# xxcclong/GNN-Computing

Measured on NVIDIA B200. Metric: gcn_layer_algorithmic_GBps, higher is better.
Workload: dtype f32

## Files before the change

### gnn-computing_b200/csrc/capi.cu

```cuda
#include <cuda_runtime.h>

#include <cstdio>
#include <cstdlib>
#include <cstring>
#include <memory>
#include <string>
#include <utility>
#include <vector>

#include "agg_kernels.cuh"
#include "edge_kernels.cuh"
#include "gnnagg.h"
#include "internal.h"

namespace gnnagg {

static thread_local std::string g_error;

int set_error(int code, const char *msg)
{
    g_error = msg ? msg : "";
    return code;
}

#define CUDA_TRY(expr)                                                                       \
    do {                                                                                     \
        cudaError_t _e = (expr);                                                             \
        if (_e != cudaSuccess) {                                                             \
            char _buf[512];                                                                  \
            snprintf(_buf, sizeof _buf, "%s:%d %s: %s", __FILE__, __LINE__, #expr, cudaGetErrorString(_e)); \
            return set_error(GNNAGG_ERR_CUDA, _buf);                                         \
        }                                                                                    \
    } while (0)

#define LAUNCH_CHECK(a)                   \
    do {                                  \
        CUDA_TRY(cudaPeekAtLastError()); \
        ++(a)->launches;                  \
    } while (0)

template <class T>
struct DevBuf {
    T *p = nullptr;
    size_t cap = 0;

    DevBuf() = default;
    DevBuf(const DevBuf &) = delete;
    DevBuf(DevBuf &&o) noexcept : p(o.p), cap(o.cap) { o.p = nullptr, o.cap = 0; }
    DevBuf &operator=(DevBuf o) noexcept
    {
        std::swap(p, o.p), std::swap(cap, o.cap);
        return *this;
    }
    ~DevBuf()
    {
        if (p) cudaFree(p);
    }

    int ensure(size_t need)
    {
        if (need <= cap && p) return GNNAGG_OK;
        if (p) CUDA_TRY(cudaFree(p));
        p = nullptr;
        cap = 0;
        CUDA_TRY(cudaMalloc((void **)&p, (need ? need : 1) * sizeof(T)));
        cap = need;
        return GNNAGG_OK;
    }
    void adopt(T *q) { *this = DevBuf(), p = q; }
};

template <int N>
struct Events {
    cudaEvent_t e[N] = {};

    Events() = default;
    Events(const Events &) = delete;
    ~Events()
    {
        for (cudaEvent_t x : e)
            if (x) cudaEventDestroy(x);
    }
    cudaEvent_t operator[](int i) const { return e[i]; }
    bool created() const { return e[0] != nullptr; }
    int create(unsigned flags)
    {
        for (cudaEvent_t &x : e) CUDA_TRY(cudaEventCreateWithFlags(&x, flags));
        return GNNAGG_OK;
    }
};

struct SideStream {
    cudaStream_t stream = nullptr;
    Events<9> ev;

    SideStream() = default;
    SideStream(const SideStream &) = delete;
    ~SideStream()
    {
        if (stream) cudaStreamDestroy(stream);
    }
    int ensure()
    {
        if (stream) return GNNAGG_OK;
        CUDA_TRY(cudaStreamCreateWithFlags(&stream, cudaStreamNonBlocking));
        return ev.create(cudaEventDisableTiming);
    }
};

static inline int64_t cdiv(int64_t a, int64_t b) { return (a + b - 1) / b; }

static bool pdl_enabled()
{
    static const bool on = [] {
        const char *e = getenv("GNNAGG_PDL");
        return e ? atoi(e) != 0 : true;
    }();
    return on;
}

template <class... KArgs, class... Args>
static void launch_dep(void (*kernel)(KArgs...), unsigned grid, unsigned block, cudaStream_t st, Args &&...args)
{
    cudaLaunchConfig_t cfg{};
    cfg.gridDim = dim3(grid);
    cfg.blockDim = dim3(block);
    cfg.stream = st;
    cudaLaunchAttribute attr[1];
    attr[0].id = cudaLaunchAttributeProgrammaticStreamSerialization;
    attr[0].val.programmaticStreamSerializationAllowed = 1;
    cfg.attrs = attr;
    cfg.numAttrs = pdl_enabled() ? 1 : 0;
    cudaLaunchKernelEx(&cfg, kernel, KArgs(args)...);
}

}

using namespace gnnagg;

constexpr int kMaxSlices = 16;
constexpr double kLocalityMinL2Multiples = 8.0;
constexpr double kLocalitySliceL2Multiples = 2.5;
constexpr double kLocalityMinDegree = 20.0;
constexpr int kLocalityMaxAuto = 4;
constexpr int64_t kMergeMinEdges = 4000000;
constexpr double kMergeMinFraction = 0.10;

struct LongRows {
    int item_edges = 0, count = 0;
    DevBuf<int> list;
    DevBuf<int2> records;
};

struct View {
    gnnagg_aggregator *root = nullptr;
    const int *d_ptr = nullptr, *d_idx = nullptr;
    const float *d_val = nullptr;
    int n = 0, m = 0;
    const int *d_item_row = nullptr;
    int num_items = 0;
    int warp_edges = 0;
    bool records = false;
    const int *out_row = nullptr;
    DevBuf<float> carry, carry_den, den_row;
    std::vector<LongRows> long_rows;
    const int *h_ptr_user = nullptr;
    std::vector<int> h_ptr;
};

struct Slices {
    struct Slice {
        DevBuf<int> item_row, c_ptr, out_row;
        View v;
    };
    DevBuf<int> ptr, idx, perm;
    DevBuf<float> val;
    uint64_t val_gen = 0;
    int off[kMaxSlices] = {0}, cnt[kMaxSlices] = {0};
    int width = 0;
    std::vector<Slice> slice;
};

struct Transpose {
    DevBuf<int> ptr, idx, perm, item_row;
    DevBuf<float> val;
    uint64_t val_gen = 0;
    View v;
};

struct Merged {
    DevBuf<int> ptr, idx, start, item_row;
    DevBuf<float> val;
    uint64_t val_gen = 0;
    View v;
};

struct Schedule {
    int kind = GNNAGG_SCHED_NOP;
    int num_target = 0, edges = 0, items = 0;
    DevBuf<int> ptr, target, perm, item_row, own_idx;
    DevBuf<float> own_val;
    const int *idx = nullptr;
    const float *val = nullptr;
};

struct gnnagg_aggregator : View {
    int64_t launches = 0;
    uint64_t val_gen = 0;
    DevBuf<int> item_row;
    DevBuf<float> newval, ax;
    DevBuf<float> st_in, st_out, st_w, st_att;
    Schedule sched;
    std::unique_ptr<Transpose> tr;
    DevBuf<float2> bwd_c, bwd_wt, bwd_part, bwd_carry;
    DevBuf<float> bwd_t;
    SideStream copy, in;
    int host_slices = 0;
    std::unique_ptr<Slices> host;
    int loc_slices = 0;
    std::unique_ptr<Slices> loc;
    int merge_mode = 0;
    int merge_auto = -1;
    std::unique_ptr<Merged> mg;
    bool prof = false;
    Events<5> ev;
};

#define PROF_RECORD(a, i, st)                                   \
    do {                                                        \
        if ((a)->prof) CUDA_TRY(cudaEventRecord((a)->ev[i], st)); \
    } while (0)

namespace gnnagg {

static EdgeParams edge_params(const View &v)
{
    EdgeParams g;
    g.ptr = v.d_ptr;
    g.idx = v.d_idx;
    g.item_row = v.d_item_row;
    g.num_rows = v.n;
    g.num_edges = v.m;
    g.num_items = v.num_items;
    return g;
}

int build_item_rows_device(const int *d_ptr, int rows, int edges, int **out, int *items, cudaStream_t st)
{
    *items = (int)cdiv(edges, kFineItem);
    *out = nullptr;
    CUDA_TRY(cudaMalloc((void **)out, (size_t)(*items ? *items : 1) * sizeof(int)));
    if (*items > 0) {
        item_row_kernel<<<(unsigned)cdiv(*items, 256), 256, 0, st>>>(d_ptr, rows, edges, *out, *items);
        CUDA_TRY(cudaPeekAtLastError());
    }
    return GNNAGG_OK;
}

static int item_table(DevBuf<int> &buf, const int *d_ptr, int rows, int edges, int *items, cudaStream_t st)
{
    int *out = nullptr;
    const int rc = build_item_rows_device(d_ptr, rows, edges, &out, items, st);
    buf.adopt(out);
    return rc;
}

__global__ void gather_val_kernel(const float *__restrict__ val, const int *__restrict__ perm, float *__restrict__ out,
                                  int count)
{
    const int i = blockIdx.x * blockDim.x + threadIdx.x;
    if (i < count) out[i] = __ldg(val + __ldg(perm + i));
}

__global__ void scatter_val_kernel(const float *__restrict__ in, const int *__restrict__ perm, float *__restrict__ out, int count)
{
    const int i = blockIdx.x * blockDim.x + threadIdx.x;
    if (i < count) out[__ldg(perm + i)] = __ldg(in + i);
}

__global__ void merge_val_kernel(const float *__restrict__ val, const int *__restrict__ start, float *__restrict__ out,
                                 int runs)
{
    const int k = blockIdx.x * blockDim.x + threadIdx.x;
    if (k >= runs) return;
    const int end = __ldg(start + k + 1);
    double s = 0.0;
    for (int e = __ldg(start + k); e < end; ++e) s += (double)__ldg(val + e);
    out[k] = (float)s;
}

static int check_feat(int F)
{
    if (F < 4 || F > 1024 || (F & 3)) return set_error(GNNAGG_ERR_ARG, "feat must be a multiple of 4 in [4,1024]");
    return GNNAGG_OK;
}

static inline int lanes_for(int F) { return F <= 32 ? 8 : (F <= 64 ? 16 : 32); }

constexpr int64_t kSmallGraphEdges = 4000000;

static inline int warp_edges_for(const View &v, int64_t num_edges)
{
    if (v.warp_edges) return v.warp_edges;
    return num_edges < kSmallGraphEdges ? 128 : kWarpEdges;
}
static inline int item_edges_for(const View &v, int F, int64_t num_edges)
{
    return warp_edges_for(v, num_edges) / (32 / lanes_for(F));
}

using AggKernel = void (*)(const AggParams);

template <int MODE, bool SCHED, bool XBF16 = false>
static AggKernel agg_kernel_for(int WE, int F)
{
    if (WE == 128)
        return F <= 32 ? agg_kernel<8, 1, MODE, SCHED, 128, XBF16>
             : F <= 64 ? agg_kernel<16, 1, MODE, SCHED, 128, XBF16>
             : F <= 128 ? agg_kernel<32, 1, MODE, SCHED, 128, XBF16>
                        : agg_kernel<32, 2, MODE, SCHED, 128, XBF16>;
    return F <= 32 ? agg_kernel<8, 1, MODE, SCHED, kWarpEdges, XBF16>
         : F <= 64 ? agg_kernel<16, 1, MODE, SCHED, kWarpEdges, XBF16>
         : F <= 128 ? agg_kernel<32, 1, MODE, SCHED, kWarpEdges, XBF16>
                    : agg_kernel<32, 2, MODE, SCHED, kWarpEdges, XBF16>;
}
template <int MODE, bool SCHED>
static AggKernel agg_kernel_for(int WE, int F, bool xbf16)
{
    if constexpr (MODE == kModeGCN)
        if (xbf16) return agg_kernel_for<MODE, SCHED, true>(WE, F);
    return agg_kernel_for<MODE, SCHED>(WE, F);
}

template <class K>
static void preload(K kernel)
{
    cudaFuncAttributes attr;
    if (cudaFuncGetAttributes(&attr, kernel) != cudaSuccess) cudaGetLastError();
}

static const LongRows *long_rows_of(View &v, const AggParams &p, int EB, cudaStream_t st)
{
    for (const LongRows &e : v.long_rows)
        if (e.item_edges == EB) return &e;
    LongRows e;
    e.item_edges = EB;
    const int64_t items = cdiv(v.m, EB);
    if (e.list.ensure((size_t)v.m / ((size_t)kFixChunk * EB) + 2)) return nullptr;
    int *counter = nullptr;
    if (cudaMalloc((void **)&counter, sizeof(int)) != cudaSuccess || e.records.ensure((size_t)items + 1)) {
        cudaFree(counter);
        set_error(GNNAGG_ERR_CUDA, "out of device memory");
        return nullptr;
    }
    cudaMemsetAsync(counter, 0, sizeof(int), st);
    long_rows_kernel<<<(unsigned)cdiv(v.n, 256), 256, 0, st>>>(v.d_ptr, v.n, EB, e.list.p, counter);
    fixup_records_kernel<<<(unsigned)cdiv(items, 256), 256, 0, st>>>(p, EB, items, e.records.p);
    cudaError_t err = cudaMemcpyAsync(&e.count, counter, sizeof(int), cudaMemcpyDeviceToHost, st);
    if (err == cudaSuccess) err = cudaStreamSynchronize(st);
    cudaFree(counter);
    if (err != cudaSuccess) {
        set_error(GNNAGG_ERR_CUDA, cudaGetErrorString(err));
        return nullptr;
    }
    v.root->launches += 2;
    v.long_rows.push_back(std::move(e));
    return &v.long_rows.back();
}

template <int MODE, bool SCHED>
static int launch_agg(View &v, AggParams p, cudaStream_t st, bool xbf16 = false)
{
    if (p.row_hi == 0 && p.edge_hi == 0) {
        p.row_lo = 0, p.row_hi = p.num_rows, p.edge_lo = 0, p.edge_hi = p.num_edges;
    }
    if (p.edge_hi <= p.edge_lo) return GNNAGG_OK;
    gnnagg_aggregator *a = v.root;
    if (v.records) PROF_RECORD(a, 1, st);
    const int WE = warp_edges_for(v, p.num_edges);
    const int64_t first = (int64_t)(p.edge_lo / WE) * WE;
    const unsigned grid = (unsigned)cdiv(p.edge_hi - first, (int64_t)WE * kCtaWarps);
    const AggKernel kernel = agg_kernel_for<MODE, SCHED>(WE, p.F, xbf16);
    if (MODE == kModeGATBWD || MODE == kModeGATBWD2)
        launch_dep(kernel, grid, kCtaThreads, st, p);
    else
        kernel<<<grid, kCtaThreads, 0, st>>>(p);
    LAUNCH_CHECK(a);
    if (v.records) PROF_RECORD(a, 2, st);
    if (!SCHED && !mode_emits_edges(MODE)) {
        const int EB = item_edges_for(v, p.F, p.num_edges);
        const int64_t items = cdiv(p.num_edges, EB);
        const int64_t range_items = cdiv(p.edge_hi, EB) - p.edge_lo / EB;
        if (range_items > 1) {
            const LongRows *lr = long_rows_of(v, p, EB, st);
            if (!lr) return GNNAGG_ERR_CUDA;
            const int lanes = lanes_for(p.F);
            launch_dep(agg_fixup_kernel<MODE>, (unsigned)cdiv(range_items * lanes, 256), 256, st, p, EB, items,
                       (const int2 *)lr->records.p, lanes);
            LAUNCH_CHECK(a);
            if (lr->count > 0) {
                launch_dep(agg_fixup_long_kernel<MODE>, (unsigned)cdiv(lr->count, 8), 256, st, p, EB, (const int *)lr->list.p,
                           lr->count);
                LAUNCH_CHECK(a);
            }
        }
    }
    return GNNAGG_OK;
}

static int aligned16(const void *p) { return (reinterpret_cast<uintptr_t>(p) & 15) == 0; }

struct GatherX {
    const void *p;
    bool bf16;
    GatherX(const float *x) : p(x), bf16(false) {}
    GatherX(const uint16_t *x) : p(x), bf16(true) {}
    int elem_bytes() const { return bf16 ? 2 : 4; }
};

static int check_xy(const GatherX &X, const float *Y)
{
    if (X.bf16) {
        if ((reinterpret_cast<uintptr_t>(X.p) & 7) || !aligned16(Y))
            return set_error(GNNAGG_ERR_ARG, "X (bf16) must be 8-byte aligned and Y 16-byte aligned");
    } else if (!aligned16(X.p) || !aligned16(Y)) {
        return set_error(GNNAGG_ERR_ARG, "X and Y must be 16-byte aligned");
    }
    return GNNAGG_OK;
}

static void set_view(AggParams &p, const View &v)
{
    p.ptr = v.d_ptr;
    p.idx = v.d_idx;
    p.item_row = v.d_item_row;
    p.num_rows = v.n;
    p.num_edges = v.m;
    p.num_fine_items = v.num_items;
}
static void set_sched(AggParams &p, const gnnagg_aggregator *a)
{
    p.ptr = a->sched.ptr.p;
    p.idx = a->sched.idx;
    p.target = a->sched.target.p;
    p.item_row = a->sched.item_row.p;
    p.num_rows = a->sched.num_target;
    p.num_edges = a->sched.edges;
    p.num_fine_items = a->sched.items;
}

static int sched_prologue(gnnagg_aggregator *a, float *Y, int F, cudaStream_t st, AggParams &p)
{
    if (a->sched.kind == GNNAGG_SCHED_NOP) return set_error(GNNAGG_ERR_STATE, "scheduled run before schedule");
    CUDA_TRY(cudaMemsetAsync(Y, 0, (size_t)a->n * F * sizeof(float), st));
    set_sched(p, a);
    return GNNAGG_OK;
}

static int gcn_run_core(View &v, GatherX X, float *Y, int F, int scheduled, cudaStream_t st, int accumulate = 0,
                        int row_lo = 0, int row_hi = -1, int edge_lo = 0, int edge_hi = 0)
{
    if (v.n == 0) return GNNAGG_OK;
    if (!X.p || !Y) return set_error(GNNAGG_ERR_ARG, "gnnagg_gcn_run: NULL argument");
    if (int rc = check_feat(F)) return rc;
    if (int rc = check_xy(X, Y)) return rc;
    if (!v.d_val && v.m > 0) return set_error(GNNAGG_ERR_STATE, "gnnagg_gcn_run: edge values not set (gnnagg_set_val)");
    AggParams p{};
    p.X = X.p;
    p.Y = Y;
    p.F = F;
    if (scheduled) {
        if (int rc = sched_prologue(v.root, Y, F, st, p)) return rc;
        if (p.num_edges == 0) return GNNAGG_OK;
        p.val = v.root->sched.val;
        p.bulk_ok = aligned16(p.idx) && aligned16(p.val);
        return launch_agg<kModeGCN, true>(v, p, st, X.bf16);
    }
    if (v.m == 0) {
        if (!accumulate) CUDA_TRY(cudaMemsetAsync(Y, 0, (size_t)v.n * F * sizeof(float), st));
        return GNNAGG_OK;
    }
    const int EB = item_edges_for(v, F, v.m);
    if (int rc = v.carry.ensure((size_t)cdiv(v.m, EB) * F)) return rc;
    set_view(p, v);
    p.accumulate = accumulate;
    p.out_row = v.out_row;
    p.val = v.d_val;
    p.carry = v.carry.p;
    p.bulk_ok = aligned16(p.idx) && aligned16(p.val);
    if (row_hi >= 0) {
        p.row_lo = row_lo, p.row_hi = row_hi, p.edge_lo = edge_lo, p.edge_hi = edge_hi;
        if (row_hi <= row_lo) return GNNAGG_OK;
        if (edge_hi <= edge_lo) {
            if (!accumulate) CUDA_TRY(cudaMemsetAsync(Y + (size_t)row_lo * F, 0, (size_t)(row_hi - row_lo) * F * sizeof(float), st));
            return GNNAGG_OK;
        }
    }
    return launch_agg<kModeGCN, false>(v, p, st, X.bf16);
}

static int host_ptr(View &v, const int **out)
{
    if (v.h_ptr_user) {
        *out = v.h_ptr_user;
        return GNNAGG_OK;
    }
    if (v.h_ptr.empty()) {
        v.h_ptr.resize((size_t)v.n + 1);
        CUDA_TRY(cudaMemcpy(v.h_ptr.data(), v.d_ptr, v.h_ptr.size() * sizeof(int), cudaMemcpyDeviceToHost));
    }
    *out = v.h_ptr.data();
    return GNNAGG_OK;
}

static void row_chunks(const int *hp, int n, int m, int chunks, int *bounds)
{
    bounds[0] = 0;
    for (int c = 1; c < chunks; ++c) {
        const int64_t target = (int64_t)m * c / chunks;
        int lo = bounds[c - 1], hi = n;
        while (lo < hi) {
            const int mid = lo + (hi - lo) / 2;
            if (hp[mid] >= target)
                hi = mid;
            else
                lo = mid + 1;
        }
        bounds[c] = lo;
    }
    bounds[chunks] = n;
}

static int gat_run_core(gnnagg_aggregator *a, const float *X, const float *att, float *Y, int F, float slope,
                        int scheduled, cudaStream_t st)
{
    if (a && a->n == 0) return GNNAGG_OK;
    if (!a || !X || !Y || !att) return set_error(GNNAGG_ERR_ARG, "gnnagg_gat_run: NULL argument");
    if (int rc = check_feat(F)) return rc;
    if (!aligned16(X) || !aligned16(Y)) return set_error(GNNAGG_ERR_ARG, "X and Y must be 16-byte aligned");
    if (int rc = a->den_row.ensure((size_t)a->n)) return rc;
    AggParams p{};
    p.X = X;
    p.Y = Y;
    p.att = att;
    p.F = F;
    p.slope = slope;
    p.den_row = a->den_row.p;
    if (scheduled) {
        if (int rc = sched_prologue(a, Y, F, st, p)) return rc;
        if (p.num_edges == 0) return GNNAGG_OK;
        CUDA_TRY(cudaMemsetAsync(a->den_row.p, 0, (size_t)a->n * sizeof(float), st));
        if (int rc = a->newval.ensure((size_t)a->sched.edges)) return rc;
        p.newval = a->newval.p;
        p.bulk_ok = aligned16(p.idx);
        if (int rc = launch_agg<kModeGAT, true>(*a, p, st)) return rc;
        const int64_t total4 = (int64_t)a->n * F / 4;
        gat_scale_kernel<<<(unsigned)cdiv(total4, 256), 256, 0, st>>>(Y, a->den_row.p, F, total4);
        LAUNCH_CHECK(a);
        return GNNAGG_OK;
    }
    if (a->m == 0) {
        CUDA_TRY(cudaMemsetAsync(Y, 0, (size_t)a->n * F * sizeof(float), st));
        return GNNAGG_OK;
    }
    const int EB = item_edges_for(*a, F, a->m);
    if (int rc = a->carry.ensure((size_t)cdiv(a->m, EB) * F)) return rc;
    if (int rc = a->carry_den.ensure((size_t)cdiv(a->m, EB))) return rc;
    set_view(p, *a);
    p.carry = a->carry.p;
    p.carry_den = a->carry_den.p;
    p.bulk_ok = aligned16(p.idx);
    return launch_agg<kModeGAT, false>(*a, p, st);
}

static int mlp_run_core(gnnagg_aggregator *a, const float *P, float *Y, int F, int scheduled, cudaStream_t st)
{
    AggParams p{};
    p.X = P;
    p.P = P;
    p.Y = Y;
    p.F = F;
    if (scheduled) {
        if (int rc = sched_prologue(a, Y, F, st, p)) return rc;
        if (p.num_edges == 0) return GNNAGG_OK;
        p.bulk_ok = aligned16(p.idx);
        return launch_agg<kModeMLP, true>(*a, p, st);
    }
    if (a->m == 0) {
        CUDA_TRY(cudaMemsetAsync(Y, 0, (size_t)a->n * F * sizeof(float), st));
        return GNNAGG_OK;
    }
    const int EB = item_edges_for(*a, F, a->m);
    if (int rc = a->carry.ensure((size_t)cdiv(a->m, EB) * F)) return rc;
    set_view(p, *a);
    p.carry = a->carry.p;
    p.bulk_ok = aligned16(p.idx);
    return launch_agg<kModeMLP, false>(*a, p, st);
}

static int ensure_slices(gnnagg_aggregator *a, std::unique_ptr<Slices> &set, int want, cudaStream_t st, bool compact = false)
{
    if (!set || (int)set->slice.size() != want) {
        set.reset();
        auto s = std::make_unique<Slices>();
        const int width = (int)cdiv(a->n, want);
        int *sp = nullptr, *si = nullptr, *sq = nullptr;
        if (int rc = source_slices_build_device(a->d_ptr, a->d_idx, a->d_item_row, a->num_items, a->n, a->m, want, width,
                                                &sp, &si, &sq, s->off, s->cnt, st))
            return rc;
        s->ptr.adopt(sp), s->idx.adopt(si), s->perm.adopt(sq);
        if (s->val.ensure((size_t)a->m + 4 * (size_t)want))
            return set_error(GNNAGG_ERR_CUDA, "host pipeline: out of device memory for the source slices");
        s->slice.resize(want);
        for (int c = 0; c < want; ++c) {
            Slices::Slice &sl = s->slice[c];
            View &v = sl.v;
            v.root = a;
            v.d_ptr = s->ptr.p + (size_t)c * ((size_t)a->n + 1);
            v.d_idx = s->idx.p + s->off[c];
            v.d_val = s->val.p + s->off[c];
            v.n = a->n;
            v.m = s->cnt[c];
            v.warp_edges = a->warp_edges ? a->warp_edges : (a->m < kSmallGraphEdges ? 128 : kWarpEdges);
            if (compact && c > 0) {
                int *cp = nullptr, *rows = nullptr;
                const int rc = compact_rows_device(v.d_ptr, a->n, &cp, &rows, &v.n, st);
                if (rc) return rc;
                sl.c_ptr.adopt(cp), sl.out_row.adopt(rows);
                v.d_ptr = cp;
                v.out_row = rows;
            }
            if (int rc = item_table(sl.item_row, v.d_ptr, v.n, v.m, &v.num_items, st)) return rc;
            v.d_item_row = sl.item_row.p;
        }
        s->width = width;
        set = std::move(s);
        a->launches += 6 + 3 * want;
    }
    if (set->val_gen != a->val_gen) {
        for (int c = 0; c < want; ++c) {
            if (set->cnt[c] == 0) continue;
            gather_val_kernel<<<(unsigned)cdiv(set->cnt[c], 256), 256, 0, st>>>(a->d_val, set->perm.p + set->off[c],
                                                                                set->val.p + set->off[c], set->cnt[c]);
            LAUNCH_CHECK(a);
        }
        set->val_gen = a->val_gen;
    }
    return GNNAGG_OK;
}


static int locality_slices_for(const gnnagg_aggregator *a, int F, int x_elem_bytes)
{
    if (a->loc_slices >= 1) return a->loc_slices < kMaxSlices ? a->loc_slices : kMaxSlices;
    int dev = 0, l2 = 0;
    if (cudaGetDevice(&dev) != cudaSuccess || cudaDeviceGetAttribute(&l2, cudaDevAttrL2CacheSize, dev) != cudaSuccess || l2 <= 0)
        return 1;
    const double x_bytes = (double)x_elem_bytes * (double)a->n * F;
    if (x_bytes < kLocalityMinL2Multiples * (double)l2 || a->m < kSmallGraphEdges) return 1;
    if ((double)a->m < kLocalityMinDegree * (double)a->n) return 1;
    int S = (int)(x_bytes / (kLocalitySliceL2Multiples * (double)l2) + 0.999);
    return S < 2 ? 1 : (S > kLocalityMaxAuto ? kLocalityMaxAuto : S);
}

static int gcn_run_sliced(gnnagg_aggregator *a, GatherX X, float *Y, int F, int S, cudaStream_t st, int accumulate)
{
    if (int rc = ensure_slices(a, a->loc, S, st, true)) return rc;
    PROF_RECORD(a, 1, st);
    for (int c = 0; c < S; ++c)
        if (int rc = gcn_run_core(a->loc->slice[c].v, X, Y, F, 0, st, accumulate || c > 0)) return rc;
    PROF_RECORD(a, 2, st);
    return GNNAGG_OK;
}

static int prof_agg_empty(gnnagg_aggregator *a, cudaStream_t st)
{
    if (a->prof) {
        CUDA_TRY(cudaEventRecord(a->ev[1], st));
        CUDA_TRY(cudaEventRecord(a->ev[2], st));
    }
    return GNNAGG_OK;
}

static int merged_view(gnnagg_aggregator *a, cudaStream_t st, View **out);

static int gcn_run_impl(gnnagg_aggregator *a, GatherX X, float *Y, int F, int scheduled, cudaStream_t st,
                        bool last = true, int accumulate = 0)
{
    if (!a) return set_error(GNNAGG_ERR_ARG, "gnnagg_gcn_run: NULL argument");
    PROF_RECORD(a, 0, st);
    if (int rc = prof_agg_empty(a, st)) return rc;
    int S = 1;
    if (!scheduled && a->n > 0 && a->m > 0 && X.p && Y && check_feat(F) == GNNAGG_OK && a->d_val)
        S = locality_slices_for(a, F, X.elem_bytes());
    if (S > 1) {
        if (int rc = check_xy(X, Y)) return rc;
        if (int rc = gcn_run_sliced(a, X, Y, F, S, st, accumulate)) return rc;
    } else {
        View *t = a;
        if (!scheduled)
            if (int rc = merged_view(a, st, &t)) return rc;
        if (int rc = gcn_run_core(*t, X, Y, F, scheduled, st, accumulate)) return rc;
    }
    PROF_RECORD(a, 3, st);
    if (last) PROF_RECORD(a, 4, st);
    return GNNAGG_OK;
}

static int gat_run_impl(gnnagg_aggregator *a, const float *X, const float *att, float *Y, int F, float slope,
                        int scheduled, cudaStream_t st)
{
    if (a) {
        PROF_RECORD(a, 0, st);
        if (int rc = prof_agg_empty(a, st)) return rc;
    }
    if (int rc = gat_run_core(a, X, att, Y, F, slope, scheduled, st)) return rc;
    PROF_RECORD(a, 3, st);
    PROF_RECORD(a, 4, st);
    return GNNAGG_OK;
}

template <int SRC = kSumArray>
static int rowsum_impl(View &v, const float *in, float *out, cudaStream_t st, int ostride = 1, float slope = 0.f)
{
    if (v.m == 0) {
        if (ostride == 1)
            CUDA_TRY(cudaMemsetAsync(out, 0, (size_t)v.n * sizeof(float), st));
        else if (v.n > 0)
            CUDA_TRY(cudaMemset2DAsync(out, (size_t)ostride * sizeof(float), 0, sizeof(float), (size_t)v.n, st));
        return GNNAGG_OK;
    }
    const int64_t items = cdiv(v.m, kRowsumItem);
    if (int rc = v.carry_den.ensure((size_t)items)) return rc;
    const EdgeParams g = edge_params(v);
    const unsigned grid = (unsigned)cdiv(items, 256);
    rowsum_kernel<SRC><<<grid, 256, 0, st>>>(g, in, slope, out, v.carry_den.p, ostride);
    LAUNCH_CHECK(v.root);
    if (items > 1) {
        rowsum_fixup_kernel<1><<<grid, 256, 0, st>>>(g, out, v.carry_den.p, ostride);
        LAUNCH_CHECK(v.root);
        if (items > kRowsumChunk + 1) {
            rowsum_fixup_kernel<2><<<grid, 256, 0, st>>>(g, out, v.carry_den.p, ostride);
            LAUNCH_CHECK(v.root);
        }
    }
    return GNNAGG_OK;
}

static bool merged_in_use(const gnnagg_aggregator *a)
{
    return a->mg && (a->merge_mode == 2 || (a->merge_mode == 0 && a->merge_auto == 1));
}

static int ensure_merged(gnnagg_aggregator *a, cudaStream_t st)
{
    if (a->merge_mode == 1 || a->n == 0 || a->m == 0) return GNNAGG_OK;
    if (a->merge_mode == 0 && a->merge_auto < 0) {
        int mm = a->m;
        if (a->m >= kMergeMinEdges) {
            if (int rc = merge_count_device(a->d_ptr, a->d_idx, a->n, a->m, &mm, st)) return rc;
            a->launches += 2;
        }
        a->merge_auto = (double)(a->m - mm) >= kMergeMinFraction * (double)a->m && a->m >= kMergeMinEdges;
    }
    if (a->merge_mode == 0 && a->merge_auto == 0) return GNNAGG_OK;
    if (!a->mg) {
        auto g = std::make_unique<Merged>();
        int *mp = nullptr, *mi = nullptr, *ms = nullptr;
        View &v = g->v;
        if (int rc = merge_build_device(a->d_ptr, a->d_idx, a->n, a->m, &mp, &mi, &ms, &v.m, st)) return rc;
        g->ptr.adopt(mp), g->idx.adopt(mi), g->start.adopt(ms);
        a->launches += 5;
        if (g->val.ensure((size_t)v.m)) return set_error(GNNAGG_ERR_CUDA, "merged view: out of device memory");
        v.root = a;
        v.d_ptr = mp;
        v.d_idx = mi;
        v.d_val = g->val.p;
        v.n = a->n;
        v.records = true;
        if (int rc = item_table(g->item_row, mp, v.n, v.m, &v.num_items, st)) return rc;
        v.d_item_row = g->item_row.p;
        a->launches += v.num_items > 0;
        a->mg = std::move(g);
    }
    return GNNAGG_OK;
}

static int merged_view(gnnagg_aggregator *a, cudaStream_t st, View **out)
{
    *out = a;
    if (a->merge_mode == 1 || !a->d_val) return GNNAGG_OK;
    if (int rc = ensure_merged(a, st)) return rc;
    if (!merged_in_use(a)) return GNNAGG_OK;
    Merged &g = *a->mg;
    if (g.val_gen != a->val_gen) {
        merge_val_kernel<<<(unsigned)cdiv(g.v.m, 256), 256, 0, st>>>(a->d_val, g.start.p, g.val.p, g.v.m);
        LAUNCH_CHECK(a);
        g.val_gen = a->val_gen;
    }
    g.v.warp_edges = a->warp_edges;
    *out = &g.v;
    return GNNAGG_OK;
}

static int gcn_layer_impl(gnnagg_aggregator *a, GatherX X, const float *W, float *H, float *AX, int feat_in, int feat_out,
                          int scheduled, void *stream)
{
    if (!a || !X.p || !W || !H) return set_error(GNNAGG_ERR_ARG, "gnnagg_gcn_layer: NULL argument");
    float *ax = AX;
    if (!ax) {
        if (int rc = a->ax.ensure((size_t)a->n * feat_in)) return rc;
        ax = a->ax.p;
    }
    if (int rc = gcn_run_impl(a, X, ax, feat_in, scheduled, (cudaStream_t)stream, false)) return rc;
    if (a->n > 0) {
        if (int rc = dense_nn_launch(ax, W, H, a->n, feat_out, feat_in, stream)) return rc;
        a->launches += 2;
    }
    PROF_RECORD(a, 4, (cudaStream_t)stream);
    return GNNAGG_OK;
}

static int gcn_backward_impl(gnnagg_aggregator *a, GatherX dY, float *dX, int feat, cudaStream_t st)
{
    if (!a || !dY.p || !dX) return set_error(GNNAGG_ERR_ARG, "gnnagg_gcn_backward: NULL argument");
    if (!a->tr) return set_error(GNNAGG_ERR_STATE, "gnnagg_gcn_backward: gnnagg_transpose_build has not run");
    if (!a->d_val && a->m > 0) return set_error(GNNAGG_ERR_STATE, "gnnagg_gcn_backward: edge values not set (gnnagg_set_val)");
    Transpose &t = *a->tr;
    if (t.val_gen != a->val_gen) {
        if (a->m > 0) {
            gather_val_kernel<<<(unsigned)cdiv(a->m, 256), 256, 0, st>>>(a->d_val, t.perm.p, t.val.p, a->m);
            LAUNCH_CHECK(a);
        }
        t.val_gen = a->val_gen;
    }
    return gcn_run_core(t.v, dY, dX, feat, 0, st);
}

}

extern "C" {

int gnnagg_version(void) { return 100; }
const char *gnnagg_last_error(void) { return g_error.c_str(); }

int gnnagg_device_info(int *sm_count, int *cc_major, int *cc_minor, char *name, int name_len)
{
    int dev = 0;
    CUDA_TRY(cudaGetDevice(&dev));
    cudaDeviceProp prop;
    CUDA_TRY(cudaGetDeviceProperties(&prop, dev));
    if (sm_count) *sm_count = prop.multiProcessorCount;
    if (cc_major) *cc_major = prop.major;
    if (cc_minor) *cc_minor = prop.minor;
    if (name && name_len > 0) {
        strncpy(name, prop.name, (size_t)name_len - 1);
        name[name_len - 1] = 0;
    }
    return GNNAGG_OK;
}

int gnnagg_create(const int *d_ptr, const int *d_idx, const int *h_ptr, const int *h_idx, int num_v, int num_e,
                  gnnagg_aggregator **out)
{
    const int rc = gnnagg_create_on(d_ptr, d_idx, h_ptr, h_idx, num_v, num_e, out, nullptr);
    if (rc == GNNAGG_OK) CUDA_TRY(cudaStreamSynchronize(0));
    return rc;
}

int gnnagg_create_on(const int *d_ptr, const int *d_idx, const int *h_ptr, const int *h_idx, int num_v, int num_e,
                     gnnagg_aggregator **out, void *stream)
{
    if (!out || !d_ptr || (num_e > 0 && !d_idx) || num_v < 0 || num_e < 0)
        return set_error(GNNAGG_ERR_ARG, "gnnagg_create: bad argument");
    std::unique_ptr<gnnagg_aggregator> a(new gnnagg_aggregator());
    a->root = a.get();
    a->records = true;
    a->d_ptr = d_ptr;
    a->d_idx = d_idx;
    a->h_ptr_user = h_ptr;
    a->n = num_v;
    a->m = num_e;
    if (int rc = item_table(a->item_row, d_ptr, num_v, num_e, &a->num_items, (cudaStream_t)stream)) return rc;
    a->d_item_row = a->item_row.p;
    a->launches += a->num_items > 0;
    *out = a.release();
    return GNNAGG_OK;
}

int gnnagg_destroy(gnnagg_aggregator *a)
{
    delete a;
    return GNNAGG_OK;
}

int gnnagg_set_val(gnnagg_aggregator *a, const float *d_val)
{
    const int rc = gnnagg_set_val_on(a, d_val, nullptr);
    if (rc == GNNAGG_OK && a->sched.perm.p) CUDA_TRY(cudaStreamSynchronize(0));
    return rc;
}

int gnnagg_set_val_on(gnnagg_aggregator *a, const float *d_val, void *stream)
{
    if (!a) return set_error(GNNAGG_ERR_ARG, "gnnagg_set_val: NULL aggregator");
    a->d_val = d_val;
    ++a->val_gen;
    Schedule &s = a->sched;
    if (s.kind == GNNAGG_SCHED_NOP) return GNNAGG_OK;
    if (s.perm.p) {
        if (int rc = s.own_val.ensure((size_t)s.edges)) return rc;
        s.val = s.own_val.p;
        if (d_val && s.edges > 0) {
            gather_val_kernel<<<(unsigned)cdiv(s.edges, 256), 256, 0, (cudaStream_t)stream>>>(d_val, s.perm.p, s.own_val.p, s.edges);
            LAUNCH_CHECK(a);
        }
    } else {
        s.val = d_val;
    }
    return GNNAGG_OK;
}

int gnnagg_schedule_apply(gnnagg_aggregator *a, int kind, const int *params, int nparams, int total_num_v)
{
    if (!a || !params || nparams < 1) return set_error(GNNAGG_ERR_ARG, "gnnagg_schedule_apply: bad argument");
    if (kind == GNNAGG_SCHED_LOCALITY_NEIGHBOR_GROUPING && nparams < 2)
        return set_error(GNNAGG_ERR_ARG, "locality_neighbor_grouping needs {par_num, neighbor_num}");
    int par = 0, ng = 0;
    if (kind == GNNAGG_SCHED_NEIGHBOR_GROUPING)
        ng = params[0];
    else if (kind == GNNAGG_SCHED_LOCALITY)
        par = params[0];
    else if (kind == GNNAGG_SCHED_LOCALITY_NEIGHBOR_GROUPING)
        par = params[0], ng = params[1];
    else
        return set_error(GNNAGG_ERR_ARG, "gnnagg_schedule_apply: unknown kind");

    int *sp = nullptr, *si = nullptr, *stg = nullptr, *sperm = nullptr, nt = 0, se = 0;
    if (int rc = schedule_build_device(kind, a->d_ptr, a->d_idx, a->d_item_row, a->num_items, a->n, a->m, par, ng,
                                       total_num_v, &sp, &si, &stg, &sperm, &nt, &se, 0))
        return rc;
    Schedule &s = a->sched;
    s = Schedule();
    s.kind = kind;
    s.num_target = nt;
    s.edges = se;
    s.ptr.adopt(sp), s.target.adopt(stg), s.perm.adopt(sperm), s.own_idx.adopt(si);
    s.idx = si ? si : a->d_idx;
    if (int rc = item_table(s.item_row, sp, nt, se, &s.items, 0)) return rc;
    a->launches += s.items > 0;
    if (int rc = gnnagg_set_val(a, a->d_val)) return rc;
    CUDA_TRY(cudaStreamSynchronize(0));
    return GNNAGG_OK;
}

int gnnagg_schedule_kind(const gnnagg_aggregator *a) { return a ? a->sched.kind : GNNAGG_SCHED_NOP; }

int gnnagg_sched_to_csr_order(gnnagg_aggregator *a, const float *in_sched, float *out_csr, void *stream)
{
    if (!a || (a->m > 0 && (!in_sched || !out_csr))) return set_error(GNNAGG_ERR_ARG, "gnnagg_sched_to_csr_order: NULL argument");
    if (a->m == 0) return GNNAGG_OK;
    cudaStream_t st = (cudaStream_t)stream;
    if (!a->sched.perm.p) {
        if (in_sched != out_csr) CUDA_TRY(cudaMemcpyAsync(out_csr, in_sched, (size_t)a->m * sizeof(float), cudaMemcpyDeviceToDevice, st));
        return GNNAGG_OK;
    }
    if (in_sched == out_csr) return set_error(GNNAGG_ERR_ARG, "gnnagg_sched_to_csr_order: in place is not possible after a locality schedule");
    if (a->sched.edges != a->m)
        return set_error(GNNAGG_ERR_STATE, "gnnagg_sched_to_csr_order: the schedule dropped edges (sources outside the slice range)");
    scatter_val_kernel<<<(unsigned)cdiv(a->m, 256), 256, 0, st>>>(in_sched, a->sched.perm.p, out_csr, a->m);
    LAUNCH_CHECK(a);
    return GNNAGG_OK;
}

int gnnagg_num_target(const gnnagg_aggregator *a) { return a ? a->sched.num_target : 0; }
const int *gnnagg_sched_dev_ptr(const gnnagg_aggregator *a) { return a ? a->sched.ptr.p : nullptr; }
const int *gnnagg_sched_dev_idx(const gnnagg_aggregator *a) { return a ? a->sched.idx : nullptr; }
const int *gnnagg_sched_dev_target(const gnnagg_aggregator *a) { return a ? a->sched.target.p : nullptr; }
const float *gnnagg_sched_dev_val(const gnnagg_aggregator *a) { return a ? a->sched.val : nullptr; }
const float *gnnagg_gat_edge_weights(const gnnagg_aggregator *a) { return a ? a->newval.p : nullptr; }
int64_t gnnagg_launch_count(const gnnagg_aggregator *a) { return a ? a->launches : 0; }

int gnnagg_set_warp_edges(gnnagg_aggregator *a, int warp_edges)
{
    if (!a || (warp_edges != 0 && warp_edges != 128 && warp_edges != 512))
        return set_error(GNNAGG_ERR_ARG, "gnnagg_set_warp_edges: 0, 128 or 512");
    a->warp_edges = warp_edges;
    if (a->tr) a->tr->v.warp_edges = warp_edges;
    return GNNAGG_OK;
}

int gnnagg_set_locality_slices(gnnagg_aggregator *a, int slices)
{
    if (!a || slices < 0 || slices > kMaxSlices) return set_error(GNNAGG_ERR_ARG, "gnnagg_set_locality_slices: 0 (automatic), 1 (off) .. 16");
    a->loc_slices = slices;
    return GNNAGG_OK;
}

int gnnagg_set_merge_duplicates(gnnagg_aggregator *a, int mode)
{
    if (!a || mode < 0 || mode > 2) return set_error(GNNAGG_ERR_ARG, "gnnagg_set_merge_duplicates: 0 (automatic), 1 (off), 2 (on)");
    a->merge_mode = mode;
    return GNNAGG_OK;
}

int gnnagg_merged_edges(gnnagg_aggregator *a)
{
    if (!a) return set_error(-1, "gnnagg_merged_edges: NULL aggregator");
    if (ensure_merged(a, nullptr) != GNNAGG_OK) return -1;
    return merged_in_use(a) ? a->mg->v.m : a->m;
}

int gnnagg_merged_dev(const gnnagg_aggregator *a, const int **ptr, const int **idx, const float **val)
{
    if (!a || !merged_in_use(a)) return set_error(GNNAGG_ERR_STATE, "gnnagg_merged_dev: the merged view is not in use");
    if (ptr) *ptr = a->mg->ptr.p;
    if (idx) *idx = a->mg->idx.p;
    if (val) *val = a->mg->val.p;
    return GNNAGG_OK;
}

int gnnagg_profile_enable(gnnagg_aggregator *a, int on)
{
    if (!a) return set_error(GNNAGG_ERR_ARG, "gnnagg_profile_enable: NULL aggregator");
    if (on && !a->ev.created())
        if (int rc = a->ev.create(cudaEventDefault)) return rc;
    a->prof = on != 0;
    return GNNAGG_OK;
}

int gnnagg_profile_read(gnnagg_aggregator *a, float *ms)
{
    if (!a || !ms || !a->ev.created()) return set_error(GNNAGG_ERR_STATE, "gnnagg_profile_read: profiling not enabled");
    CUDA_TRY(cudaEventSynchronize(a->ev[4]));
    float agg = 0.f, agg_total = 0.f, dense = 0.f, total = 0.f;
    CUDA_TRY(cudaEventElapsedTime(&agg, a->ev[1], a->ev[2]));
    CUDA_TRY(cudaEventElapsedTime(&agg_total, a->ev[0], a->ev[3]));
    CUDA_TRY(cudaEventElapsedTime(&dense, a->ev[3], a->ev[4]));
    CUDA_TRY(cudaEventElapsedTime(&total, a->ev[0], a->ev[4]));
    ms[0] = agg;
    ms[1] = agg_total - agg;
    ms[2] = dense;
    ms[3] = total;
    return GNNAGG_OK;
}

int gnnagg_memcpy_d2h(void *h_dst, const void *d_src, uint64_t bytes)
{
    if (bytes == 0) return GNNAGG_OK;
    if (!h_dst || !d_src) return set_error(GNNAGG_ERR_ARG, "gnnagg_memcpy_d2h: NULL argument");
    CUDA_TRY(cudaMemcpy(h_dst, d_src, bytes, cudaMemcpyDeviceToHost));
    return GNNAGG_OK;
}

int gnnagg_prepare(gnnagg_aggregator *a, int feat, void *stream)
{
    if (!a) return set_error(GNNAGG_ERR_ARG, "gnnagg_prepare: NULL aggregator");
    if (int rc = check_feat(feat)) return rc;
    if (a->m == 0 || a->n == 0) return GNNAGG_OK;
    View *t = a;
    if (int rc = merged_view(a, (cudaStream_t)stream, &t)) return rc;
    View &v = *t;
    const int EB = item_edges_for(v, feat, v.m);
    if (int rc = v.carry.ensure((size_t)cdiv(v.m, EB) * feat)) return rc;
    preload(agg_kernel_for<kModeGCN, false>(warp_edges_for(v, v.m), feat));
    preload(agg_kernel_for<kModeGCN, false, true>(warp_edges_for(v, v.m), feat));
    preload(agg_fixup_kernel<kModeGCN>);
    preload(agg_fixup_long_kernel<kModeGCN>);
    AggParams p{};
    set_view(p, v);
    if (!long_rows_of(v, p, EB, (cudaStream_t)stream)) return GNNAGG_ERR_CUDA;
    const int *hp = nullptr;
    return host_ptr(v, &hp);
}

static int gcn_run_rows_impl(gnnagg_aggregator *a, GatherX X, float *Y, int feat, int accumulate, int row_lo, int row_hi,
                             cudaStream_t st)
{
    if (!a) return set_error(GNNAGG_ERR_ARG, "gnnagg_gcn_run_rows: NULL aggregator");
    if (row_lo < 0 || row_hi > a->n || row_lo > row_hi) return set_error(GNNAGG_ERR_ARG, "gnnagg_gcn_run_rows: bad row range");
    if (row_lo == row_hi) return GNNAGG_OK;
    View *t = a;
    if (int rc = merged_view(a, st, &t)) return rc;
    const int *hp = nullptr;
    if (int rc = host_ptr(*t, &hp)) return rc;
    return gcn_run_core(*t, X, Y, feat, 0, st, accumulate != 0, row_lo, row_hi, hp[row_lo], hp[row_hi]);
}

int gnnagg_gcn_run_rows(gnnagg_aggregator *a, const float *X, float *Y, int feat, int accumulate, int row_lo, int row_hi,
                        void *stream)
{
    return gcn_run_rows_impl(a, X, Y, feat, accumulate, row_lo, row_hi, (cudaStream_t)stream);
}

int gnnagg_gcn_run_rows_bf16(gnnagg_aggregator *a, const uint16_t *X, float *Y, int feat, int accumulate, int row_lo,
                             int row_hi, void *stream)
{
    return gcn_run_rows_impl(a, X, Y, feat, accumulate, row_lo, row_hi, (cudaStream_t)stream);
}

int gnnagg_gcn_run(gnnagg_aggregator *a, const float *X, float *Y, int feat, int scheduled, void *stream)
// ... 489 lines not shown
```

Before: 29560.

## Split dense hub block of merged graph into a blocked dense GEMM

During merged-view construction, high-degree destination rows and high in-degree source columns are ranked on the host, and a cost model picks a K×K hub block. Edges inside that block are packed into a dense partitioned matrix and handled with a gather, an FP32 tiled GEMM and a partial-sum add. The remaining edges go through the usual sparse aggregation. This replaces many irregular gathers on dense graphs with regular dense compute, at the price of a host-side preprocessing pass, extra memory for the dense block and partials, and three more launches per run.

```diff
diff --git a/gnn-computing_b200/csrc/capi.cu b/gnn-computing_b200/csrc/capi.cu
--- a/gnn-computing_b200/csrc/capi.cu
+++ b/gnn-computing_b200/csrc/capi.cu
@@ -2,7 +2,9 @@
 
 #include <cstdio>
 #include <cstdlib>
+#include <algorithm>
 #include <cstring>
+#include <numeric>
 #include <memory>
 #include <string>
 #include <utility>
@@ -145,6 +147,11 @@
 constexpr int kLocalityMaxAuto = 4;
 constexpr int64_t kMergeMinEdges = 4000000;
 constexpr double kMergeMinFraction = 0.10;
+constexpr int64_t kHubMinEntries = 16000000;
+constexpr double kHubMinPerRow = 64.0;
+constexpr int kHubPart = 512;
+constexpr int kHubMaxBlock = 4096;
+constexpr double kHubGatherPs = 0.2, kHubCellPs = 0.08;
 
 struct LongRows {
     int item_edges = 0, count = 0;
@@ -188,11 +195,22 @@
     View v;
 };
 
+struct Hub {
+    int K = 0, entries = 0;
+    DevBuf<int> rows, srcs;
+    DevBuf<int> blk_pos, blk_cell;
+    DevBuf<int> ptr, idx, pos, item_row;
+    DevBuf<float> val, A, xh, part;
+    uint64_t val_gen = 0;
+    View v;
+};
+
 struct Merged {
     DevBuf<int> ptr, idx, start, item_row;
     DevBuf<float> val;
     uint64_t val_gen = 0;
     View v;
+    std::unique_ptr<Hub> hub;
 };
 
 struct Schedule {
@@ -457,8 +475,110 @@
     return GNNAGG_OK;
 }
 
+
+__global__ void hub_val_kernel(const float *__restrict__ mval, const int *__restrict__ blk_pos, const int *__restrict__ blk_cell,
+                               float *__restrict__ A, int nb, const int *__restrict__ pos, float *__restrict__ rval, int nr)
+{
+    const int i = blockIdx.x * blockDim.x + threadIdx.x;
+    if (i < nb) A[blk_cell[i]] = mval[blk_pos[i]];
+    if (i < nr) rval[i] = mval[pos[i]];
+}
+
+__global__ void hub_gather_kernel(const void *__restrict__ X, bool bf16, const int *__restrict__ srcs, float *__restrict__ xh,
+                                  int K, int F)
+{
+    const int64_t i = (int64_t)blockIdx.x * blockDim.x + threadIdx.x;
+    if (i >= (int64_t)K * F) return;
+    const int j = (int)(i / F), f = (int)(i % F);
+    const size_t at = (size_t)srcs[j] * F + f;
+    xh[i] = bf16 ? __uint_as_float((uint32_t)static_cast<const uint16_t *>(X)[at] << 16) : static_cast<const float *>(X)[at];
+}
+
+__global__ void __launch_bounds__(256) hub_gemm_kernel(const float *__restrict__ A, const float *__restrict__ xh,
+                                                       float *__restrict__ part, int K, int F)
+{
+    __shared__ float sA[16][64 + 1], sB[16][64];
+    const int tx = threadIdx.x & 15, ty = threadIdx.x >> 4;
+    const int row0 = blockIdx.y * 64, col0 = blockIdx.x * 64, z = blockIdx.z;
+    A += (size_t)z * K * kHubPart;
+    xh += (size_t)z * kHubPart * F;
+    part += (size_t)z * K * F;
+    float acc[4][4] = {};
+    for (int k0 = 0; k0 < kHubPart; k0 += 16) {
+        for (int i = threadIdx.x; i < 64 * 16; i += 256) {
+            const int r = i >> 4, k = i & 15;
+            sA[k][r] = A[(size_t)(row0 + r) * kHubPart + k0 + k];
+            const int kb = i >> 6, c = i & 63;
+            sB[kb][c] = col0 + c < F ? xh[(size_t)(k0 + kb) * F + col0 + c] : 0.f;
+        }
+        __syncthreads();
+#pragma unroll
+        for (int k = 0; k < 16; ++k) {
+            float a[4], b[4];
+#pragma unroll
+            for (int i = 0; i < 4; ++i) a[i] = sA[k][ty * 4 + i], b[i] = sB[k][tx * 4 + i];
+#pragma unroll
+            for (int i = 0; i < 4; ++i)
+#pragma unroll
+                for (int j = 0; j < 4; ++j) acc[i][j] = fmaf(a[i], b[j], acc[i][j]);
+        }
+        __syncthreads();
+    }
+#pragma unroll
+    for (int i = 0; i < 4; ++i)
+#pragma unroll
+        for (int j = 0; j < 4; ++j)
+            if (col0 + tx * 4 + j < F) part[(size_t)(row0 + ty * 4 + i) * F + col0 + tx * 4 + j] = acc[i][j];
+}
+
+__global__ void hub_add_kernel(const float *__restrict__ part, const int *__restrict__ rows, float *__restrict__ Y, int K,
+                               int F, int parts, int lo, int hi)
+{
+    const int64_t i = (int64_t)blockIdx.x * blockDim.x + threadIdx.x;
+    if (i >= (int64_t)K * F) return;
+    const int r = rows[i / F];
+    if (r < lo || r >= hi) return;
+    float s = part[i];
+    for (int z = 1; z < parts; ++z) s += part[(size_t)z * K * F + i];
+    float *y = Y + (size_t)r * F + i % F;
+    *y += s;
+}
+
+static Hub *hub_for(View &v, int F)
+{
+    gnnagg_aggregator *a = v.root;
+    if (!a || !a->mg || &a->mg->v != &v || !a->mg->hub || F % 32 || F > 256) return nullptr;
+    return a->mg->hub.get();
+}
+
+static int gcn_run_core(View &v, GatherX X, float *Y, int F, int scheduled, cudaStream_t st, int accumulate,
+                        int row_lo, int row_hi, int edge_lo, int edge_hi);
+
+static int gcn_run_hub(View &v, Hub &h, GatherX X, float *Y, int F, cudaStream_t st, int accumulate, int row_lo, int row_hi)
+{
+    if (!X.p || !Y) return set_error(GNNAGG_ERR_ARG, "gnnagg_gcn_run: NULL argument");
+    if (int rc = check_xy(X, Y)) return rc;
+    const int lo = row_hi >= 0 ? row_lo : 0, hi = row_hi >= 0 ? row_hi : v.n;
+    if (hi <= lo) return GNNAGG_OK;
+    h.v.warp_edges = v.warp_edges;
+    if (int rc = gcn_run_core(h.v, X, Y, F, 0, st, accumulate, lo, row_hi >= 0 ? hi : -1, h.v.h_ptr[lo], h.v.h_ptr[hi]))
+        return rc;
+    gnnagg_aggregator *a = v.root;
+    const int64_t kf = (int64_t)h.K * F;
+    hub_gather_kernel<<<(unsigned)cdiv(kf, 256), 256, 0, st>>>(X.p, X.bf16, h.srcs.p, h.xh.p, h.K, F);
+    LAUNCH_CHECK(a);
+    hub_gemm_kernel<<<dim3((unsigned)cdiv(F, 64), (unsigned)(h.K / 64), (unsigned)(h.K / kHubPart)), 256, 0, st>>>(
+        h.A.p, h.xh.p, h.part.p, h.K, F);
+    LAUNCH_CHECK(a);
+    hub_add_kernel<<<(unsigned)cdiv(kf, 256), 256, 0, st>>>(h.part.p, h.rows.p, Y, h.K, F, h.K / kHubPart, lo, hi);
+    LAUNCH_CHECK(a);
+    return GNNAGG_OK;
+}
+
 static int gcn_run_core(View &v, GatherX X, float *Y, int F, int scheduled, cudaStream_t st, int accumulate = 0,
-                        int row_lo = 0, int row_hi = -1, int edge_lo = 0, int edge_hi = 0)
+                        int row_lo = 0, int row_hi = -1, int edge_lo = 0, int edge_hi = 0);
+static int gcn_run_core(View &v, GatherX X, float *Y, int F, int scheduled, cudaStream_t st, int accumulate,
+                        int row_lo, int row_hi, int edge_lo, int edge_hi)
 {
     if (v.n == 0) return GNNAGG_OK;
     if (!X.p || !Y) return set_error(GNNAGG_ERR_ARG, "gnnagg_gcn_run: NULL argument");
@@ -476,6 +596,7 @@
         p.bulk_ok = aligned16(p.idx) && aligned16(p.val);
         return launch_agg<kModeGCN, true>(v, p, st, X.bf16);
     }
+    if (Hub *h = hub_for(v, F)) return gcn_run_hub(v, *h, X, Y, F, st, accumulate, row_lo, row_hi);
     if (v.m == 0) {
         if (!accumulate) CUDA_TRY(cudaMemsetAsync(Y, 0, (size_t)v.n * F * sizeof(float), st));
         return GNNAGG_OK;
@@ -752,6 +873,92 @@
     return a->mg && (a->merge_mode == 2 || (a->merge_mode == 0 && a->merge_auto == 1));
 }
 
+static int hub_build(gnnagg_aggregator *a, Merged &g, cudaStream_t st)
+{
+    const View &mv = g.v;
+    const int n = mv.n, mm = mv.m;
+    if ((int64_t)mm < kHubMinEntries || (double)mm < kHubMinPerRow * n) return GNNAGG_OK;
+    CUDA_TRY(cudaStreamSynchronize(st));
+    std::vector<int> hp((size_t)n + 1), hi((size_t)mm);
+    CUDA_TRY(cudaMemcpy(hp.data(), mv.d_ptr, hp.size() * sizeof(int), cudaMemcpyDeviceToHost));
+    CUDA_TRY(cudaMemcpy(hi.data(), mv.d_idx, hi.size() * sizeof(int), cudaMemcpyDeviceToHost));
+    int ns = 0;
+    for (int x : hi) ns = std::max(ns, x + 1);
+    std::vector<int> indeg((size_t)ns, 0), rorder((size_t)n), sorder((size_t)ns);
+    for (int x : hi) ++indeg[x];
+    std::iota(rorder.begin(), rorder.end(), 0);
+    std::iota(sorder.begin(), sorder.end(), 0);
+    std::stable_sort(rorder.begin(), rorder.end(), [&](int x, int y) { return hp[x + 1] - hp[x] > hp[y + 1] - hp[y]; });
+    std::stable_sort(sorder.begin(), sorder.end(), [&](int x, int y) { return indeg[x] > indeg[y]; });
+    std::vector<int> rrank((size_t)n, INT32_MAX), srank((size_t)ns, INT32_MAX);
+    for (int i = 0; i < std::min(n, kHubMaxBlock); ++i) rrank[rorder[i]] = i;
+    for (int i = 0; i < std::min(ns, kHubMaxBlock); ++i) srank[sorder[i]] = i;
+    std::vector<int64_t> within((size_t)kHubMaxBlock + 1, 0);
+    for (int r = 0; r < n; ++r)
+        if (rrank[r] < kHubMaxBlock)
+            for (int e = hp[r]; e < hp[r + 1]; ++e)
+                if (srank[hi[e]] < kHubMaxBlock) ++within[std::max(rrank[r], srank[hi[e]]) + 1];
+    for (int k = 1; k <= kHubMaxBlock; ++k) within[k] += within[k - 1];
+    int K = 0;
+    double best = 0.0;
+    for (int k = kHubPart; k <= std::min(std::min(n, ns), kHubMaxBlock); k += kHubPart) {
+        const double gain = (double)within[k] * kHubGatherPs - (double)k * k * kHubCellPs;
+        if (gain > best) best = gain, K = k;
+    }
+    if (K == 0) return GNNAGG_OK;
+    auto h = std::make_unique<Hub>();
+    h->K = K;
+    std::vector<int> bpos, bcell, rptr((size_t)n + 1, 0), ridx, rpos;
+    ridx.reserve((size_t)mm - (size_t)within[K]);
+    rpos.reserve(ridx.capacity());
+    for (int r = 0; r < n; ++r) {
+        for (int e = hp[r]; e < hp[r + 1]; ++e) {
+            const int i = rrank[r], j = srank[hi[e]];
+            if (i < K && j < K) {
+                bpos.push_back(e);
+                bcell.push_back((j / kHubPart) * K * kHubPart + i * kHubPart + j % kHubPart);
+            } else {
+                ridx.push_back(hi[e]);
+                rpos.push_back(e);
+            }
+        }
+        rptr[(size_t)r + 1] = (int)ridx.size();
+    }
+    h->entries = (int)bpos.size();
+    const int nr = (int)ridx.size();
+    auto up = [&](DevBuf<int> &d, const int *src, size_t cnt) -> int {
+        if (int rc = d.ensure(cnt)) return rc;
+        if (cnt) CUDA_TRY(cudaMemcpy(d.p, src, cnt * sizeof(int), cudaMemcpyHostToDevice));
+        return GNNAGG_OK;
+    };
+    if (int rc = up(h->rows, rorder.data(), K)) return rc;
+    if (int rc = up(h->srcs, sorder.data(), K)) return rc;
+    if (int rc = up(h->blk_pos, bpos.data(), bpos.size())) return rc;
+    if (int rc = up(h->blk_cell, bcell.data(), bcell.size())) return rc;
+    if (int rc = up(h->ptr, rptr.data(), rptr.size())) return rc;
+    if (int rc = up(h->idx, ridx.data(), ridx.size())) return rc;
+    if (int rc = up(h->pos, rpos.data(), rpos.size())) return rc;
+    if (int rc = h->val.ensure((size_t)nr)) return rc;
+    if (int rc = h->A.ensure((size_t)K * K)) return rc;
+    CUDA_TRY(cudaMemsetAsync(h->A.p, 0, (size_t)K * K * sizeof(float), st));
+    if (int rc = h->xh.ensure((size_t)K * 256)) return rc;
+    if (int rc = h->part.ensure((size_t)(K / kHubPart) * K * 256)) return rc;
+    View &v = h->v;
+    v.root = a;
+    v.d_ptr = h->ptr.p;
+    v.d_idx = h->idx.p;
+    v.d_val = h->val.p;
+    v.n = n;
+    v.m = nr;
+    v.records = true;
+    v.h_ptr = std::move(rptr);
+    if (int rc = item_table(h->item_row, h->ptr.p, v.n, v.m, &v.num_items, st)) return rc;
+    v.d_item_row = h->item_row.p;
+    a->launches += v.num_items > 0;
+    g.hub = std::move(h);
+    return GNNAGG_OK;
+}
+
 static int ensure_merged(gnnagg_aggregator *a, cudaStream_t st)
 {
     if (a->merge_mode == 1 || a->n == 0 || a->m == 0) return GNNAGG_OK;
@@ -781,6 +988,7 @@
         if (int rc = item_table(g->item_row, mp, v.n, v.m, &v.num_items, st)) return rc;
         v.d_item_row = g->item_row.p;
         a->launches += v.num_items > 0;
+        if (int rc = hub_build(a, *g, st)) return rc;
         a->mg = std::move(g);
     }
     return GNNAGG_OK;
@@ -797,6 +1005,14 @@
         merge_val_kernel<<<(unsigned)cdiv(g.v.m, 256), 256, 0, st>>>(a->d_val, g.start.p, g.val.p, g.v.m);
         LAUNCH_CHECK(a);
         g.val_gen = a->val_gen;
+    }
+    if (g.hub && g.hub->val_gen != g.val_gen) {
+        Hub &h = *g.hub;
+        const int cnt = std::max(h.entries, h.v.m);
+        hub_val_kernel<<<(unsigned)cdiv(cnt, 256), 256, 0, st>>>(g.val.p, h.blk_pos.p, h.blk_cell.p, h.A.p, h.entries, h.pos.p,
+                                                                h.val.p, h.v.m);
+        LAUNCH_CHECK(a);
+        h.val_gen = g.val_gen;
     }
     g.v.warp_edges = a->warp_edges;
     *out = &g.v;
```

Result: faster. 30530, median of 6 (+3.3%).
